# nahomes-15/pointclouds-rs

Hardware: NVIDIA B200
Metric: sor_normals_points_per_sec (higher is better)
Workload: dtype f32

## Files before the change

pointclouds_rs_b200/csrc/grid_build.cu:

```cuda
#include "pcr_internal.cuh"

#include <algorithm>
#include <cstring>
#include <chrono>
#include <cmath>

namespace pcr {

namespace {

constexpr int kBuildThreads = 256;
constexpr int kItems = 4;

using FrameStats = CloudStats;

struct ProbeStats {
    double sum_log_own, sum_log_super;
};

static inline float ordered_f32(unsigned u) {
    unsigned b = (u & 0x80000000u) ? (u & 0x7fffffffu) : ~u;
    float f;
    memcpy(&f, &b, 4);
    return f;
// ... 220 lines not shown
}

struct TombLevels {
    float4 *sorted[4];
    uint32_t n[4];
    int levels;
};
__global__ void __launch_bounds__(256) tombstone_kernel(TombLevels t, const uint8_t *__restrict__ keep) {
    PCR_GRID_DEP_SYNC();
    const uint32_t i = blockIdx.x * blockDim.x + threadIdx.x;
    for (int l = 0; l < t.levels; l++) {
        if (i >= t.n[l]) continue;
        float4 p = t.sorted[l][i];
        if (!keep[__float_as_uint(p.w)]) {
            const float qnan = __int_as_float(0x7fc00000);
            p.x = p.y = p.z = qnan;
            t.sorted[l][i] = p;
        }
    }
}

constexpr int kScanThreads = 256;
constexpr int kScanItems = 16;
constexpr int kScanTile = kScanThreads * kScanItems;

__device__ __forceinline__ uint32_t block_sum_u32(uint32_t v, uint32_t *sh) {
    v = __reduce_add_sync(PCR_FULL, v);
    if ((threadIdx.x & 31) == 0) sh[threadIdx.x >> 5] = v;
    __syncthreads();
    uint32_t t = 0;
    if (threadIdx.x < kScanThreads / 32) t = sh[threadIdx.x];
    if (threadIdx.x < 32) t = __reduce_add_sync(PCR_FULL, t);
    if (threadIdx.x == 0) sh[0] = t;
    __syncthreads();
    t = sh[0];
    __syncthreads();
    return t;
}

__global__ void __launch_bounds__(kScanThreads) scan_tile_sums_kernel(const uint32_t *__restrict__ data, size_t n,
                                                                      uint32_t *__restrict__ tile_sums) {
    __shared__ uint32_t sh[kScanThreads / 32];
    size_t base = (size_t)blockIdx.x * kScanTile;
    uint32_t s = 0;
#pragma unroll
    for (int it = 0; it < kScanItems; it++) {
        size_t i = base + it * kScanThreads + threadIdx.x;
        if (i < n) s += data[i];
    }
    s = block_sum_u32(s, sh);
    if (threadIdx.x == 0) tile_sums[blockIdx.x] = s;
}

constexpr unsigned long long kScanAgg = 1ull << 32, kScanPre = 2ull << 32;

__device__ __forceinline__ uint4 scan_load4(const uint32_t *data, size_t i, size_t n, bool vec) {
    if (vec && i + 3 < n) return *reinterpret_cast<const uint4 *>(data + i);
    uint4 v;
    v.x = i < n ? data[i] : 0u;
    v.y = i + 1 < n ? data[i + 1] : 0u;
    v.z = i + 2 < n ? data[i + 2] : 0u;
    v.w = i + 3 < n ? data[i + 3] : 0u;
    return v;
}

__device__ __forceinline__ void scan_store4(uint32_t *data, size_t i, size_t n, bool vec, uint4 v) {
    if (vec && i + 3 < n) {
        *reinterpret_cast<uint4 *>(data + i) = v;
        return;
    }
    if (i < n) data[i] = v.x;
    if (i + 1 < n) data[i + 1] = v.y;
    if (i + 2 < n) data[i + 2] = v.z;
    if (i + 3 < n) data[i + 3] = v.w;
}

__device__ __forceinline__ uint32_t scan_lookback_warp0(unsigned long long *state, uint32_t tile, uint32_t epoch, uint32_t total, int lane) {
    const unsigned long long tag = (unsigned long long)epoch << 34;
    volatile unsigned long long *vs = state;
    uint32_t pre = 0;
    if (tile > 0) {
        if (lane == 0) vs[tile] = tag | kScanAgg | total;
        long long look = (long long)tile - 1;
        for (;;) {
            const long long t = look - lane;
            const bool need = t >= 0;
            unsigned long long sv = 0;
            uint32_t polls = 0;
            bool ready;
            do {
                if (need) sv = vs[t];
                ready = !need || ((sv >> 34) == epoch && ((sv >> 32) & 3ull) != 0);
                if (++polls > (1u << 26)) __trap();
            } while (!__all_sync(PCR_FULL, ready));
            const unsigned pm = __ballot_sync(PCR_FULL, need && ((sv >> 32) & 3ull) == 2ull);
            const int stop = pm ? __ffs(pm) - 1 : 32;
            pre += __reduce_add_sync(PCR_FULL, (need && lane <= stop) ? (uint32_t)sv : 0u);
            if (pm || look < 32) break;
            look -= 32;
        }
    }
    if (lane == 0) vs[tile] = tag | kScanPre | (uint32_t)(pre + total);
    return pre;
}

__global__ void __launch_bounds__(kScanThreads) scan_lookback_kernel(uint32_t *__restrict__ data, size_t n,
                                                                     unsigned long long *state, uint32_t *ticket,
                                                                     uint32_t epoch, uint32_t tiles, int vec) {
    constexpr int kWarps = kScanThreads / 32, kRows = kScanItems / 4;
    __shared__ uint32_t s_tile, s_pre;
    __shared__ uint32_t warp_tot[kWarps];
    PCR_GRID_DEP_SYNC();
    if (threadIdx.x == 0) s_tile = atomicAdd(ticket, 1u);
    __syncthreads();
    const uint32_t tile = s_tile;
    if (tile >= tiles) return;
    const int lane = threadIdx.x & 31, w = threadIdx.x >> 5;
    const size_t wbase = (size_t)tile * kScanTile + (size_t)w * (kScanItems * 32);
    uint4 v[kRows];
    uint32_t ex[kRows];
    uint32_t carry = 0;
#pragma unroll
    for (int r = 0; r < kRows; r++) {
        v[r] = scan_load4(data, wbase + (size_t)r * 128 + lane * 4, n, vec != 0);
        const uint32_t s = v[r].x + v[r].y + v[r].z + v[r].w;
        uint32_t incl = s;
#pragma unroll
        for (int o = 1; o < 32; o <<= 1) {
            uint32_t u = __shfl_up_sync(PCR_FULL, incl, o);
            if (lane >= o) incl += u;
        }
        ex[r] = carry + incl - s;
        carry += __shfl_sync(PCR_FULL, incl, 31);
    }
    if (lane == 0) warp_tot[w] = carry;
    __syncthreads();
    uint32_t woff = 0, total = 0;
#pragma unroll
    for (int j = 0; j < kWarps; j++) {
        const uint32_t t = warp_tot[j];
        if (j < w) woff += t;
        total += t;
    }
    if (w == 0) {
        const uint32_t pre = scan_lookback_warp0(state, tile, epoch, total, lane);
        if (lane == 0) s_pre = pre;
    }
    __syncthreads();
    const uint32_t base = s_pre + woff;
#pragma unroll
    for (int r = 0; r < kRows; r++) {
        uint4 o;
        o.x = base + ex[r];
        o.y = o.x + v[r].x;
        o.z = o.y + v[r].y;
        o.w = o.z + v[r].z;
// ... 4 lines not shown

__global__ void __launch_bounds__(kScanThreads) scan_apply_u64_kernel(const uint32_t *__restrict__ in,
                                                                      uint64_t *__restrict__ out, size_t n,
                                                                      const uint32_t *__restrict__ tile_sums) {
    __shared__ unsigned long long sh64[kScanThreads / 32];
    __shared__ unsigned long long warp_off[kScanThreads / 32];
    unsigned long long pre = 0;
    for (uint32_t t = threadIdx.x; t < blockIdx.x; t += kScanThreads) pre += tile_sums[t];
    for (int o = 16; o > 0; o >>= 1) pre += __shfl_xor_sync(PCR_FULL, pre, o);
    if ((threadIdx.x & 31) == 0) sh64[threadIdx.x >> 5] = pre;
    __syncthreads();
    pre = 0;
    for (int i = 0; i < kScanThreads / 32; i++) pre += sh64[i];
    __syncthreads();
    size_t base = (size_t)blockIdx.x * kScanTile + (size_t)threadIdx.x * kScanItems;
    uint32_t v[kScanItems];
    unsigned long long tsum = 0;
#pragma unroll
    for (int it = 0; it < kScanItems; it++) {
        size_t i = base + it;
        v[it] = i < n ? in[i] : 0u;
        tsum += v[it];
    }
    unsigned long long incl = tsum;
    const int lane = threadIdx.x & 31, w = threadIdx.x >> 5;
#pragma unroll
    for (int o = 1; o < 32; o <<= 1) {
        unsigned long long u = __shfl_up_sync(PCR_FULL, incl, o);
        if (lane >= o) incl += u;
    }
    if (lane == 31) warp_off[w] = incl;
    __syncthreads();
    if (threadIdx.x == 0) {
        unsigned long long acc = 0;
        for (int i = 0; i < kScanThreads / 32; i++) {
            unsigned long long t = warp_off[i];
            warp_off[i] = acc;
            acc += t;
        }
    }
    __syncthreads();
    unsigned long long run = pre + warp_off[w] + (incl - tsum);
#pragma unroll
    for (int it = 0; it < kScanItems; it++) {
        size_t i = base + it;
        if (i < n) out[i] = run;
        run += v[it];
        if (i + 1 == n) out[n] = run;
    }
}

}

static int exclusive_scan_u32_with(Ctx *ctx, uint32_t *d_data, size_t n, DevBuf &scratch, uint32_t &scan_epoch) {
    if (n == 0) return PCR_OK;
    const size_t tiles = (n + kScanTile - 1) / kScanTile;
    const size_t cap_before = scratch.cap;
    PCR_TRY(ensure(ctx, scratch, 16 + tiles * sizeof(unsigned long long)));
    if (scratch.cap != cap_before || scan_epoch >= (1u << 30) - 2) {
        PCR_CUDA(ctx, cudaMemsetAsync(scratch.p, 0, scratch.cap, ctx->stream));
        scan_epoch = 0;
    }
    const uint32_t epoch = ++scan_epoch;
    uint32_t *ticket = (uint32_t *)scratch.p;
    unsigned long long *state = (unsigned long long *)((char *)scratch.p + 16);
    const int vec = ((uintptr_t)d_data & 15) == 0;
    PCR_CUDA(ctx, launch_chained(scan_lookback_kernel, dim3((unsigned)tiles), dim3(kScanThreads), 0, ctx->stream, d_data, n, state, ticket, epoch,
                                 (uint32_t)tiles, vec));
    ctx->launches++;
    return PCR_OK;
}

int exclusive_scan_u32_dev(Ctx *ctx, uint32_t *d_data, size_t n) { return exclusive_scan_u32_with(ctx, d_data, n, ctx->b_scan, ctx->scan_epoch); }

int exclusive_scan_u64_from_u32_dev(Ctx *ctx, const uint32_t *d_in, uint64_t *d_out, size_t n) {
    if (n == 0) {
        PCR_CUDA(ctx, cudaMemsetAsync(d_out, 0, sizeof(uint64_t), ctx->stream));
        return PCR_OK;
    }
    size_t tiles = (n + kScanTile - 1) / kScanTile;
    PCR_TRY(ensure(ctx, ctx->b_misc2, tiles * sizeof(uint32_t)));
    uint32_t *tile_sums = (uint32_t *)ctx->b_misc2.p;
    scan_tile_sums_kernel<<<(unsigned)tiles, kScanThreads, 0, ctx->stream>>>(d_in, n, tile_sums);
    PCR_LAUNCH_CHECK(ctx);
    scan_apply_u64_kernel<<<(unsigned)tiles, kScanThreads, 0, ctx->stream>>>(d_in, d_out, n, tile_sums);
    PCR_LAUNCH_CHECK(ctx);
    return PCR_OK;
}

namespace {

constexpr uint64_t kMaxCellsPerFrame = 1ull << 24;
constexpr uint64_t kMaxCellsTotal = 1ull << 27;

struct FrameBox {
    double mn[3], ext[3];
    uint32_t count;
};

double occupancy_target(size_t k_hint, bool self_knn) {
    double k = k_hint ? (double)k_hint : 10.0;
    static const bool tile_off = [] {
        const char *e = getenv("PCR_KNN_TILE");
        return e && !strcmp(e, "0");
    }();
    double scale = self_knn && !tile_off && k_hint <= 24 ? 0.5 : 0.25;
    if (const char *e = getenv("PCR_OCC_SCALE")) scale = atof(e);
    return std::min(64.0, std::max(2.0, scale * k));
}

double initial_cell(const FrameBox &b, double target) {
    if (b.count == 0) return 1.0;
    double e[3] = {b.ext[0], b.ext[1], b.ext[2]};
    std::sort(e, e + 3);
    double tiny = std::max(e[2] * 1e-6, 1e-30);
    double vol = std::max(e[0], tiny) * std::max(e[1], tiny) * std::max(e[2], tiny);
    double area = std::max(e[1], tiny) * std::max(e[2], tiny);
    double h3 = std::cbrt(vol * target / b.count);
// ... 403 lines not shown
```

pointclouds_rs_b200/csrc/pcr_internal.cuh:

```cuda
#pragma once
#include <cstdlib>

#include <cuda_runtime.h>
#include <math.h>
#include <stdint.h>
#include <stdio.h>
#include <string.h>

#include <string>
#include <vector>

#include "../../include/pcr_b200.h"

namespace pcr {

struct GridDesc {
    double o[3];
    double h, inv_h;
    int32_t dims[3];
    int32_t ax[3];
    uint32_t cell_base;
    uint32_t n_cells;
    uint32_t pt_begin;
    uint32_t pt_end;
// ... 169 lines not shown

struct CloudStats {
    unsigned mn[3], mx[3];
    unsigned count;
    unsigned valid;
};

struct BuildOpts {
    const CloudStats *known_stats = nullptr;
    size_t k_hint = 0;
    bool self_knn = false;
    int n_frames = 1;
    const uint64_t *frame_offsets = nullptr;
    const uint8_t *d_mask = nullptr;
    bool transient = false;
};
int index_build_dev(Ctx *ctx, const float *dx, const float *dy, const float *dz, size_t n,
                    const BuildOpts &opts, Index **out);
void index_free(Index *ix);
int index_coarser_level(Index *ix, Index **out);
int index_finer_level(Index *ix, Index **out);

int knn_queries_dev(Index *ix, const float *dqx, const float *dqy, const float *dqz, size_t nq,
                    size_t k, uint32_t *d_idx, float *d_dist, uint32_t *d_counts);
struct SorLists {
    size_t K = 0;
    size_t stride = 0;
    uint32_t *lists = nullptr;
    uint8_t *cnt = nullptr;
    uint32_t *fallback = nullptr;
    bool initialised = false;
};
int sor_mean_dist_dev(Index *ix, size_t k, float *d_mean_d, const SorLists *keep_lists = nullptr, bool allow_shard = false);
int normals_from_lists_dev(Index *ix, size_t k, const float vp[3], const SorLists &sl, const uint8_t *d_keep, float *d_nx, float *d_ny,
                           float *d_nz,
                           const unsigned long long *d_kept0 = nullptr, unsigned long long *h_kept0 = nullptr, bool early = false);
int normals_early_fork(Ctx *ctx);
int normals_early_from_lists_dev(Index *ix, size_t k, const float vp[3], const SorLists &sl, float *d_nx, float *d_ny, float *d_nz, bool *launched);
int normals_dev(Index *ix, size_t k, const float vp[3], float *d_nx, float *d_ny, float *d_nz,
                const uint8_t *d_mask, bool allow_shard = false);
bool query_sharding_active(const Ctx *ctx, const Index *ix);
int index_shard_queries(Index *ix);
int index_apply_mask_dev(Index *ix, const uint8_t *d_keep);
int radius_count_dev(Index *ix, const float *dqx, const float *dqy, const float *dqz, size_t nq,
                     float radius, uint32_t *d_counts);
int radius_fill_dev(Index *ix, const float *dqx, const float *dqy, const float *dqz, size_t nq,
                    float radius, const uint64_t *d_offsets, uint32_t *d_idx);

int sor_threshold_mask_dev(Ctx *ctx, const float *d_mean_d, const uint32_t *d_frame_off ,
                           int n_frames, size_t n, float std_mul, uint8_t *d_keep, float *d_stats,
                           unsigned long long *d_kept, bool kept_zeroed = false );

int exclusive_scan_u32_dev(Ctx *ctx, uint32_t *d_data, size_t n_plus_1);
int exclusive_scan_u64_from_u32_dev(Ctx *ctx, const uint32_t *d_in, uint64_t *d_out, size_t n);

struct IcpArgs {
    const float *d_sx, *d_sy, *d_sz;
    size_t ns;
    const float *d_tx, *d_ty, *d_tz;
    size_t nt;
    const float *d_nx, *d_ny, *d_nz;
    pcr_icp_params params;
};
int icp_dev(Ctx *ctx, const IcpArgs &a, pcr_icp_result *result);
struct IcpBatchArgs {
    const float *d_x, *d_y, *d_z;
    size_t n;
    const uint64_t *frame_offsets;
    size_t n_frames;
    const float *d_nx, *d_ny, *d_nz;
    const uint32_t *pairs;
    size_t n_pairs;
    pcr_icp_params params;
};
int icp_batch_dev(Ctx *ctx, const IcpBatchArgs &a, pcr_icp_result *results);
int find_correspondences_dev(Index *target, const float *dsx, const float *dsy, const float *dsz,
                             size_t ns, float max_distance, uint32_t *d_tgt, float *d_dist);
int apply_transform_dev(Ctx *ctx, const float *dx, const float *dy, const float *dz, size_t n,
                        const float R[9], const float t[3], float *ox, float *oy, float *oz);

int cluster_labels_dev(Ctx *ctx, const float *dx, const float *dy, const float *dz, size_t n, float threshold, uint32_t *d_labels,
                       const uint32_t *d_frame_off = nullptr, int n_frames = 1);
size_t clusters_from_labels(const uint32_t *labels, size_t n, size_t min_size, size_t max_size, uint32_t *offsets, uint32_t *indices,
                            std::vector<uint32_t> &scratch);
int cluster_labels_batch_dev(Ctx *ctx, const float *dx, const float *dy, const float *dz, const uint64_t *frame_offsets, size_t n_frames,
                             float threshold, uint32_t *d_labels);
int euclidean_cluster_batch_dev(Ctx *ctx, const float *dx, const float *dy, const float *dz, const uint64_t *frame_offsets, size_t n_frames,
                                float threshold, size_t min_size, size_t max_size, uint32_t *d_offsets, uint32_t *d_indices,
                                uint64_t *cluster_offsets, size_t *total);

int voxel_downsample_dev(Ctx *ctx, const float *dx, const float *dy, const float *dz, size_t n, float voxel, float *d_ox, float *d_oy,
                         float *d_oz, size_t *n_out, CloudStats *stats_out = nullptr ,
                         bool allow_guess = true );
int voxel_downsample_batch_dev(Ctx *ctx, const float *dx, const float *dy, const float *dz, const uint64_t *frame_offsets,
                               size_t n_frames, float voxel, float *d_ox, float *d_oy, float *d_oz, uint64_t *out_offsets);
int radix_sort_pairs_dev(Ctx *ctx, unsigned long long **keys, uint32_t **vals, unsigned long long **keys_alt, uint32_t **vals_alt,
                         size_t n, int bits, uint32_t *d_hist);
size_t radix_sort_hist_words(size_t n);
int bits_for(uint64_t range);

int ransac_plane_samples_dev(Ctx *ctx, const float *dx, const float *dy, const float *dz, size_t n, float threshold,
                             const uint32_t *h_samples, size_t m, float model_out[4], uint32_t *d_inliers, size_t *n_inliers);
int ransac_plane_samples_batch_dev(Ctx *ctx, const float *dx, const float *dy, const float *dz, const uint64_t *frame_offsets,
                                   size_t n_frames, float threshold, const uint32_t *h_samples, const uint64_t *sample_offsets,
                                   float *models_out, uint32_t *d_inliers, uint64_t *inlier_offsets);

// ... 34 lines not shown
    cfg.attrs = at;
    cfg.numAttrs = off ? 0 : 1;
    return cudaLaunchKernelEx(&cfg, kernel, static_cast<KArgs>(args)...);
}

#define PCR_FULL 0xffffffffu
#define PCR_EMPTY_KEY 0x7f80000100000000ull

__device__ __forceinline__ float dist2_exact(float ax, float ay, float az, float bx, float by, float bz) {
    float dx = __fsub_rn(ax, bx), dy = __fsub_rn(ay, by), dz = __fsub_rn(az, bz);
    float s = __fmul_rn(dx, dx);
    s = __fadd_rn(s, __fmul_rn(dy, dy));
    s = __fadd_rn(s, __fmul_rn(dz, dz));
    return s;
}

__device__ __forceinline__ unsigned long long make_key(float d2, uint32_t idx) {
    return ((unsigned long long)__float_as_uint(d2) << 32) | idx;
}
__device__ __forceinline__ float key_d2(unsigned long long k) { return __uint_as_float((uint32_t)(k >> 32)); }
__device__ __forceinline__ uint32_t key_idx(unsigned long long k) { return (uint32_t)k; }

__device__ __forceinline__ bool finite3(float a, float b, float c) { return isfinite(a) && isfinite(b) && isfinite(c); }
__device__ __forceinline__ unsigned f32_ordered(float f) {
    unsigned u = __float_as_uint(f);
    return (u & 0x80000000u) ? ~u : (u | 0x80000000u);
}

__device__ __forceinline__ float pick_axis(int ax, float x, float y, float z) { return ax == 0 ? x : (ax == 1 ? y : z); }

__device__ __forceinline__ int cell_coord(const GridDesc &g, int j, float v, double *frac) {
    double t = ((double)v - g.o[j]) * g.inv_h;
    double f = floor(t);
    f = fmin(fmax(f, 0.0), (double)(g.dims[j] - 1));
    if (frac) *frac = t - f;
    return (int)f;
}

__device__ __forceinline__ uint32_t cell_linear(const GridDesc &g, int c0, int c1, int c2) {
    return g.cell_base + ((uint32_t)c0 * (uint32_t)g.dims[1] + (uint32_t)c1) * (uint32_t)g.dims[2] + (uint32_t)c2;
}

__device__ __forceinline__ int frame_of(const uint32_t *__restrict__ off, int n_frames, uint32_t i) {
    if (n_frames <= 1) return 0;
    int lo = 0, hi = n_frames - 1;
    while (lo < hi) {
        int mid = (lo + hi + 1) >> 1;
        if (off[mid] <= i) lo = mid;
        else hi = mid - 1;
    }
    return lo;
}

#endif

}
```

pointclouds_rs_b200/csrc/voxel.cu:

```cuda
#include "pcr_internal.cuh"

#include <algorithm>

namespace pcr {

namespace {

constexpr int kSortRounds = 8;
constexpr int kSortTile = 32 * kSortRounds;
constexpr int kSortWarps = 4;

struct VoxHeader {
    unsigned mn_c[3], mx[3];
    unsigned count;
    unsigned outside;
    unsigned total;
    unsigned tall;
    unsigned pad[6];
};
constexpr uint32_t kTallColumn = 256;
constexpr uint32_t kLocalColumn = 32;
static_assert(sizeof(VoxHeader) == 64, "header layout");

struct VoxRange {
// ... 196 lines not shown
        return;
    }
    if (vid[i + 1] != vid[i]) start[vid[i]] = i;
}

__global__ void __launch_bounds__(128) vox_mean_kernel(const float *__restrict__ x, const float *__restrict__ y, const float *__restrict__ z,
                                                       const uint32_t *__restrict__ vals, const uint32_t *__restrict__ start,
                                                       const uint32_t *__restrict__ n_vox_dev, float *__restrict__ ox,
                                                       float *__restrict__ oy, float *__restrict__ oz) {
    const uint32_t v = blockIdx.x * blockDim.x + threadIdx.x;
    if (v >= *n_vox_dev) return;
    const uint32_t b = start[v], e = start[v + 1];
    float sx = 0.f, sy = 0.f, sz = 0.f;
    for (uint32_t i = b; i < e; i++) {
        const uint32_t p = vals[i];
        sx = __fadd_rn(sx, x[p]);
        sy = __fadd_rn(sy, y[p]);
        sz = __fadd_rn(sz, z[p]);
    }
    const float denom = (float)(e - b);
    ox[v] = __fdiv_rn(sx, denom);
    oy[v] = __fdiv_rn(sy, denom);
    oz[v] = __fdiv_rn(sz, denom);
}

__global__ void __launch_bounds__(256) vox_col_count_kernel(const float *__restrict__ x, const float *__restrict__ y,
                                                            const float *__restrict__ z, size_t n, float voxel, int mn0, int mn1,
                                                            int mn2, unsigned long long nx, unsigned long long ny,
                                                            unsigned long long nz, uint32_t nyc, int ys, uint32_t *__restrict__ count,
                                                            uint32_t *__restrict__ col_of, uint32_t *__restrict__ rank_of,
                                                            uint32_t *__restrict__ outside) {
    const size_t i = (size_t)blockIdx.x * blockDim.x + threadIdx.x;
    if (i >= n) return;
    const float px = x[i], py = y[i], pz = z[i];
    if (!finite3(px, py, pz)) {
        col_of[i] = 0xffffffffu;
        return;
    }
    const int kx = vox_cell(px, voxel), ky = vox_cell(py, voxel), kz = vox_cell(pz, voxel);
    if ((unsigned long long)((long long)kx - mn0) >= nx || (unsigned long long)((long long)ky - mn1) >= ny ||
        (unsigned long long)((long long)kz - mn2) >= nz) {
        col_of[i] = 0xffffffffu;
        *outside = 1u;
        return;
    }
    const uint32_t col = (uint32_t)(kx - mn0) * nyc + ((uint32_t)(ky - mn1) >> ys);
    col_of[i] = col;
    rank_of[i] = atomicAdd(&count[col], 1u);
}

__global__ void __launch_bounds__(256) vox_col_scatter_kernel(const float *__restrict__ y, const float *__restrict__ z, size_t n,
                                                              float voxel, int mn1, int mn2, int ys,
                                                              const uint32_t *__restrict__ start, const uint32_t *__restrict__ col_of,
                                                              const uint32_t *__restrict__ rank_of, unsigned long long *__restrict__ members) {
    PCR_GRID_DEP_SYNC();
    const size_t i = (size_t)blockIdx.x * blockDim.x + threadIdx.x;
    if (i >= n) return;
    const uint32_t col = col_of[i];
    if (col == 0xffffffffu) return;
    const uint32_t ylo = (uint32_t)(vox_cell(y[i], voxel) - mn1) & ((1u << ys) - 1u);
    const uint32_t hi = (ys ? ylo << (32 - ys) : 0u) | (uint32_t)(vox_cell(z[i], voxel) - mn2);
    members[start[col] + rank_of[i]] = ((unsigned long long)hi << 32) | (uint32_t)i;
}

__global__ void __launch_bounds__(256) vox_col_sort_kernel(const uint32_t *__restrict__ col_of, const uint32_t *__restrict__ rank_of,
                                                           size_t n, const uint32_t *__restrict__ start,
                                                           unsigned long long *__restrict__ members, uint32_t *__restrict__ nvox,
                                                           unsigned *__restrict__ tall) {
    PCR_GRID_DEP_SYNC();
    const size_t i = (size_t)blockIdx.x * blockDim.x + threadIdx.x;
    if (i >= n) return;
    const uint32_t c = col_of[i];
    if (c == 0xffffffffu || rank_of[i] != 0u) return;
    const uint32_t b = start[c], e = start[c + 1], m = e - b;
    if (m > kTallColumn) {
        *tall = 1u;
        return;
    }
    unsigned long long *a = members + b;
    if (m == 1) {
        nvox[b] = 1u;
        return;
    }
    if (m <= kLocalColumn) {
        unsigned long long loc[kLocalColumn];
        for (uint32_t j0 = 0; j0 < m; j0 += 8) {
            unsigned long long t[8];
#pragma unroll
            for (int u = 0; u < 8; u++) t[u] = a[min(j0 + u, m - 1)];
#pragma unroll
            for (int u = 0; u < 8; u++)
                if (j0 + u < m) loc[j0 + u] = t[u];
        }
        for (uint32_t i = 1; i < m; i++) {
            const unsigned long long v = loc[i];
            uint32_t j = i;
            while (j > 0 && loc[j - 1] > v) {
                loc[j] = loc[j - 1];
                j--;
            }
            loc[j] = v;
        }
        uint32_t nv = 1;
        a[0] = loc[0];
        for (uint32_t i = 1; i < m; i++) {
            a[i] = loc[i];
            nv += (uint32_t)(loc[i] >> 32) != (uint32_t)(loc[i - 1] >> 32) ? 1u : 0u;
        }
        nvox[b] = nv;
        return;
    } else {
        for (uint32_t s0 = m / 2; s0-- > 0;) {
            uint32_t root = s0;
            for (;;) {
                uint32_t ch = 2 * root + 1;
// ... 65 lines not shown
                cnt = 0;
                cur = kz;
            }
            sx = __fadd_rn(sx, X[u]);
            sy = __fadd_rn(sy, Y[u]);
            sz = __fadd_rn(sz, Z[u]);
            cnt++;
        }
    }
    const float denom = (float)cnt;
    ox[v] = __fdiv_rn(sx, denom);
    oy[v] = __fdiv_rn(sy, denom);
    oz[v] = __fdiv_rn(sz, denom);
}

__global__ void __launch_bounds__(256) vox_out_stats_kernel(const float *__restrict__ x, const float *__restrict__ y,
                                                            const float *__restrict__ z, const uint32_t *__restrict__ d_n,
                                                            VoxHeader *hdr) {
    PCR_GRID_DEP_SYNC();
    const uint32_t n = *d_n;
    if (blockIdx.x == 0 && threadIdx.x == 0) hdr->total = n;
    unsigned mn_c[3] = {0u, 0u, 0u}, mx[3] = {0u, 0u, 0u}, cnt = 0;
    for (uint32_t i = blockIdx.x * blockDim.x + threadIdx.x; i < n; i += gridDim.x * blockDim.x) {
        const float px = x[i], py = y[i], pz = z[i];
        if (!finite3(px, py, pz)) continue;
        const unsigned u[3] = {f32_ordered(px), f32_ordered(py), f32_ordered(pz)};
        for (int a = 0; a < 3; a++) {
            mn_c[a] = max(mn_c[a], ~u[a]);
            mx[a] = max(mx[a], u[a]);
        }
        cnt++;
    }
    for (int a = 0; a < 3; a++) {
        mn_c[a] = __reduce_max_sync(PCR_FULL, mn_c[a]);
        mx[a] = __reduce_max_sync(PCR_FULL, mx[a]);
    }
    cnt = __reduce_add_sync(PCR_FULL, cnt);
    __shared__ unsigned s_mn[3], s_mx[3], s_cnt;
    if (threadIdx.x == 0) {
        s_mn[0] = s_mn[1] = s_mn[2] = 0u;
        s_mx[0] = s_mx[1] = s_mx[2] = 0u;
        s_cnt = 0;
    }
    __syncthreads();
    if ((threadIdx.x & 31) == 0 && cnt) {
        for (int a = 0; a < 3; a++) {
            atomicMax(&s_mn[a], mn_c[a]);
            atomicMax(&s_mx[a], mx[a]);
        }
        atomicAdd(&s_cnt, cnt);
    }
    __syncthreads();
    if (threadIdx.x == 0 && s_cnt) {
        for (int a = 0; a < 3; a++) {
            atomicMax(&hdr->mn_c[a], s_mn[a]);
            atomicMax(&hdr->mx[a], s_mx[a]);
        }
        atomicAdd(&hdr->count, s_cnt);
    }
}

__global__ void __launch_bounds__(256) vox_frame_starts_kernel(const unsigned long long *__restrict__ keys, const uint32_t *__restrict__ vals,
                                                               uint32_t m, int fshift ,
                                                               const uint32_t *__restrict__ frame_off, int n_frames,
                                                               const uint32_t *__restrict__ vid, uint32_t *__restrict__ out_off) {
    const uint32_t i = blockIdx.x * blockDim.x + threadIdx.x;
    if (i > m) return;
    auto frame = [&](uint32_t j) { return fshift >= 0 ? (int)(keys[j] >> fshift) : frame_of(frame_off, n_frames, vals[j]); };
    const int hi = i < m ? frame(i) : n_frames;
    const int lo = i > 0 ? frame(i - 1) : -1;
    for (int f = lo + 1; f <= hi; f++) out_off[f] = vid[i];
}

}

int bits_for(uint64_t range) {
    int b = 0;
    while (b < 64 && (1ull << b) < range) b++;
    return b;
}

size_t radix_sort_hist_words(size_t n) { return (size_t)256 * ((n + kSortTile - 1) / kSortTile) + 1; }

int radix_sort_pairs_dev(Ctx *ctx, unsigned long long **keys, uint32_t **vals, unsigned long long **keys_alt, uint32_t **vals_alt,
                         size_t n, int bits, uint32_t *d_hist ) {
    if (n == 0) return PCR_OK;
    const uint32_t n_tiles = (uint32_t)((n + kSortTile - 1) / kSortTile);
    const unsigned blocks = (n_tiles + kSortWarps - 1) / kSortWarps;
    for (int shift = 0; shift < bits; shift += 8) {
        sort_hist_kernel<<<blocks, 32 * kSortWarps, 0, ctx->stream>>>(*keys, n, shift, n_tiles, d_hist);
        PCR_LAUNCH_CHECK(ctx);
        PCR_TRY(exclusive_scan_u32_dev(ctx, d_hist, (size_t)256 * n_tiles + 1));
        sort_scatter_kernel<<<blocks, 32 * kSortWarps, 0, ctx->stream>>>(*keys, *vals, n, shift, n_tiles, d_hist, *keys_alt, *vals_alt);
        PCR_LAUNCH_CHECK(ctx);
        std::swap(*keys, *keys_alt);
        std::swap(*vals, *vals_alt);
    }
    return PCR_OK;
}

int voxel_downsample_dev(Ctx *ctx, const float *dx, const float *dy, const float *dz, size_t n, float voxel, float *d_ox, float *d_oy,
                         float *d_oz, size_t *n_out, CloudStats *stats_out, bool allow_guess) {
    *n_out = 0;
    if (stats_out) stats_out->valid = 0;
    if (n == 0) return PCR_OK;
    if (n > 0x7fffffffull) return fail(ctx, PCR_ERR_UNSUPPORTED, "clouds above 2^31 points are not supported");
    cudaStream_t st = ctx->stream;
    TimeScope ts(ctx, kTagOther);
    PCR_TRY(ensure(ctx, ctx->b_small, 4096));
    PCR_TRY(ensure_pinned(ctx, 4096));
    VoxRange *d_range = (VoxRange *)ctx->b_small.p;
    uint32_t *d_nvox = (uint32_t *)((char *)ctx->b_small.p + 256);
    VoxRange *h_range = (VoxRange *)ctx->pinned;
    auto &vc = ctx->vox_cache;
    static const bool no_guess = getenv("PCR_NO_VOXEL_GUESS") != nullptr;
    const bool guessed = allow_guess && !no_guess && ctx->frame_stream && vc.valid && vc.voxel == voxel && vc.uses < 32;
    uint32_t m;
    if (guessed) {
        vc.uses++;
        for (int a = 0; a < 3; a++) {
            h_range->mn[a] = vc.mn[a];
            h_range->mx[a] = vc.mx[a];
        }
        m = (uint32_t)n;
    } else {
        vox_init_kernel<<<1, 1, 0, st>>>(d_range, 1);
        PCR_LAUNCH_CHECK(ctx);
        const unsigned bx = (unsigned)std::min<size_t>((n + 255) / 256, (size_t)ctx->sm_count * 2);
        vox_range_kernel<<<bx, 256, 0, st>>>(dx, dy, dz, nullptr, n, voxel, d_range);
        PCR_LAUNCH_CHECK(ctx);
        PCR_CUDA(ctx, cudaMemcpyAsync(h_range, d_range, sizeof(VoxRange), cudaMemcpyDeviceToHost, st));
        PCR_MARK("voxel: wait for range");
        PCR_CUDA(ctx, cudaStreamSynchronize(st));
        PCR_MARK("voxel: got range");
        m = h_range->finite;
        if (m == 0) return PCR_OK;
        vc.valid = false;
        if (ctx->frame_stream) {
            bool ok = true;
            for (int a = 0; a < 3; a++) {
                const long long ext = (long long)h_range->mx[a] - (long long)h_range->mn[a] + 1;
                const long long pad = std::max<long long>(2, ext >> vc.pad_shift);
                const long long lo = (long long)h_range->mn[a] - pad, hi = (long long)h_range->mx[a] + pad;
                if (lo < -2147483647ll || hi > 2147483646ll) ok = false;
                vc.mn[a] = (int)lo;
                vc.mx[a] = (int)hi;
            }
            vc.valid = ok;
            vc.voxel = voxel;
            vc.uses = 0;
        }
    }
    {
        const uint64_t nx = (uint64_t)((int64_t)h_range->mx[0] - (int64_t)h_range->mn[0]) + 1;
        const uint64_t ny = (uint64_t)((int64_t)h_range->mx[1] - (int64_t)h_range->mn[1]) + 1;
        const uint64_t nz = (uint64_t)((int64_t)h_range->mx[2] - (int64_t)h_range->mn[2]) + 1;
        int ys = 0;
        static const int ys_max = getenv("PCR_VOXEL_YS") ? atoi(getenv("PCR_VOXEL_YS")) : 0;
        while (ys < ys_max && nz < (1ull << (32 - (ys + 1))) && nx * ((ny + (2ull << ys) - 1) >> (ys + 1)) >= (uint64_t)m) ys++;
        while (ys < 4 && nz < (1ull << (32 - (ys + 1))) && nx * ((ny + (1ull << ys) - 1) >> ys) > (1ull << 24)) ys++;
        const uint64_t nyc64 = (ny + (1ull << ys) - 1) >> ys;
        const uint64_t n_cols64 = nx * nyc64;
        static const bool no_cols = getenv("PCR_VOXEL_RADIX") != nullptr;
        if (!no_cols && nx < (1ull << 31) && ny < (1ull << 31) && nz < (1ull << (32 - ys)) && n_cols64 <= (1ull << 24) &&
            n_cols64 <= 64ull * m + 65536ull) {
            const uint32_t n_cols = (uint32_t)n_cols64;
            const size_t tab = (sizeof(uint32_t) * ((size_t)n_cols + 1) + 15) & ~(size_t)15;
            const size_t tab_v = (sizeof(uint32_t) * ((size_t)n + 1) + 15) & ~(size_t)15;
            const size_t o_count = sizeof(VoxHeader), o_nvox = o_count + tab;
            const size_t o_col = (o_nvox + tab_v + 15) & ~(size_t)15;
            const size_t o_rank = o_col + sizeof(uint32_t) * n;
            const size_t o_mem = (o_rank + sizeof(uint32_t) * n + 15) & ~(size_t)15;
            PCR_TRY(ensure(ctx, ctx->b_table, o_mem + sizeof(unsigned long long) * n));
            char *base = (char *)ctx->b_table.p;
            VoxHeader *d_hdr = (VoxHeader *)base;
            uint32_t *count = (uint32_t *)(base + o_count), *nvox = (uint32_t *)(base + o_nvox);
            uint32_t *col_of = (uint32_t *)(base + o_col), *rank_of = (uint32_t *)(base + o_rank);
            unsigned long long *members = (unsigned long long *)(base + o_mem);
            PCR_CUDA(ctx, cudaMemsetAsync(base, 0, o_nvox + tab_v, st));
            const unsigned nbp = (unsigned)((n + 255) / 256);
            vox_col_count_kernel<<<nbp, 256, 0, st>>>(dx, dy, dz, n, voxel, h_range->mn[0], h_range->mn[1], h_range->mn[2], nx, ny, nz,
                                                      (uint32_t)nyc64, ys, count, col_of, rank_of, &d_hdr->outside);
            PCR_LAUNCH_CHECK(ctx);
            PCR_TRY(exclusive_scan_u32_dev(ctx, count, (size_t)n_cols + 1));
            PCR_CUDA(ctx, launch_chained(vox_col_scatter_kernel, dim3(nbp), dim3(256), 0, st, dy, dz, n, voxel, h_range->mn[1], h_range->mn[2], ys,
                                         count, col_of, rank_of, members));
            PCR_CUDA(ctx, launch_chained(vox_col_sort_kernel, dim3(nbp), dim3(256), 0, st, col_of, rank_of, n, count, members, nvox, &d_hdr->tall));
            ctx->launches += 2;
            PCR_TRY(exclusive_scan_u32_dev(ctx, nvox, n + 1));
            PCR_CUDA(ctx, launch_chained(vox_col_emit_kernel, dim3(nbp), dim3(256), 0, st, dx, dy, dz, col_of, rank_of, n, count, nvox, members, d_ox,
                                         d_oy, d_oz));
            ctx->launches++;
            PCR_CUDA(ctx, launch_chained(vox_out_stats_kernel, dim3((unsigned)ctx->sm_count), dim3(256), 0, st, d_ox, d_oy, d_oz, nvox + n, d_hdr));
            ctx->launches++;
            VoxHeader *mail = (VoxHeader *)((uint32_t *)ctx->pinned + 64);
            PCR_CUDA(ctx, cudaMemcpyAsync(mail, d_hdr, sizeof(VoxHeader), cudaMemcpyDeviceToHost, st));
            PCR_MARK("voxel: wait for count");
            PCR_CUDA(ctx, cudaStreamSynchronize(st));
            PCR_MARK("voxel: got count");
            if (guessed) (mail->outside ? ctx->stat_vox_misses : ctx->stat_vox_hits)++;
            if (guessed && mail->outside) {
                vc.valid = false;
                vc.pad_shift = std::max(2, vc.pad_shift - 1);
                return voxel_downsample_dev(ctx, dx, dy, dz, n, voxel, d_ox, d_oy, d_oz, n_out, stats_out, false);
            }
            const bool tall = mail->tall != 0;
            if (tall && guessed) {
                vc.valid = false;
                return voxel_downsample_dev(ctx, dx, dy, dz, n, voxel, d_ox, d_oy, d_oz, n_out, stats_out, false);
            }
            if (!tall) *n_out = mail->total;
            if (!tall && stats_out) {
                for (int a = 0; a < 3; a++) {
                    stats_out->mn[a] = ~mail->mn_c[a];
                    stats_out->mx[a] = mail->mx[a];
                }
                stats_out->count = mail->count;
                stats_out->valid = 1;
            }
            if (!tall) return PCR_OK;
        }
    }
    if (guessed) {
        vc.valid = false;
        return voxel_downsample_dev(ctx, dx, dy, dz, n, voxel, d_ox, d_oy, d_oz, n_out, stats_out, false);
    }
    int bits[3];
    for (int a = 0; a < 3; a++) bits[a] = bits_for((uint64_t)((int64_t)h_range->mx[a] - (int64_t)h_range->mn[a]) + 1);
    const int total_bits = bits[0] + bits[1] + bits[2];
    const bool packed = total_bits <= 63;

    const size_t n_tiles = (n + kSortTile - 1) / kSortTile;
    const size_t need = 2 * sizeof(unsigned long long) * n + sizeof(uint32_t) * (2 * n + 256 * n_tiles + 1 + 2 * (n + 1)) + 1024;
    PCR_TRY(ensure(ctx, ctx->b_table, need));
    char *p = (char *)ctx->b_table.p;
    unsigned long long *kA = (unsigned long long *)p;
    p += sizeof(unsigned long long) * n;
    unsigned long long *kB = (unsigned long long *)p;
    p += sizeof(unsigned long long) * n;
    uint32_t *vA = (uint32_t *)p;
    p += sizeof(uint32_t) * n;
    uint32_t *vB = (uint32_t *)p;
    p += sizeof(uint32_t) * n;
    uint32_t *hist = (uint32_t *)p;
    p += sizeof(uint32_t) * (256 * n_tiles + 1);
    uint32_t *vid = (uint32_t *)p;
    p += sizeof(uint32_t) * (n + 1);
// ... 136 lines not shown
```

Baseline: 264.4 million.

## Replace voxel column pipeline with bucketed tile sort-emit kernel using decoupled lookback

Makes a new default voxel downsampling path that bins points into coarser xy buckets and sorts each ~1024-point tile in shared memory. A single kernel then segments voxels, averages them, assigns output offsets through a decoupled lookback scan and accumulates bounds stats. It replaces the separate sort, second scan, emit and stats kernels, cutting launches and global passes. The cost is an extra bounds array written during scatter and an O(bucket size) rank loop per point. Tiles over capacity set the tall flag and fall back.

```diff
diff --git a/pointclouds_rs_b200/csrc/grid_build.cu b/pointclouds_rs_b200/csrc/grid_build.cu
--- a/pointclouds_rs_b200/csrc/grid_build.cu
+++ b/pointclouds_rs_b200/csrc/grid_build.cu
@@ -296,8 +296,6 @@
     if (threadIdx.x == 0) tile_sums[blockIdx.x] = s;
 }
 
-constexpr unsigned long long kScanAgg = 1ull << 32, kScanPre = 2ull << 32;
-
 __device__ __forceinline__ uint4 scan_load4(const uint32_t *data, size_t i, size_t n, bool vec) {
     if (vec && i + 3 < n) return *reinterpret_cast<const uint4 *>(data + i);
     uint4 v;
@@ -317,35 +315,6 @@
     if (i + 1 < n) data[i + 1] = v.y;
     if (i + 2 < n) data[i + 2] = v.z;
     if (i + 3 < n) data[i + 3] = v.w;
-}
-
-__device__ __forceinline__ uint32_t scan_lookback_warp0(unsigned long long *state, uint32_t tile, uint32_t epoch, uint32_t total, int lane) {
-    const unsigned long long tag = (unsigned long long)epoch << 34;
-    volatile unsigned long long *vs = state;
-    uint32_t pre = 0;
-    if (tile > 0) {
-        if (lane == 0) vs[tile] = tag | kScanAgg | total;
-        long long look = (long long)tile - 1;
-        for (;;) {
-            const long long t = look - lane;
-            const bool need = t >= 0;
-            unsigned long long sv = 0;
-            uint32_t polls = 0;
-            bool ready;
-            do {
-                if (need) sv = vs[t];
-                ready = !need || ((sv >> 34) == epoch && ((sv >> 32) & 3ull) != 0);
-                if (++polls > (1u << 26)) __trap();
-            } while (!__all_sync(PCR_FULL, ready));
-            const unsigned pm = __ballot_sync(PCR_FULL, need && ((sv >> 32) & 3ull) == 2ull);
-            const int stop = pm ? __ffs(pm) - 1 : 32;
-            pre += __reduce_add_sync(PCR_FULL, (need && lane <= stop) ? (uint32_t)sv : 0u);
-            if (pm || look < 32) break;
-            look -= 32;
-        }
-    }
-    if (lane == 0) vs[tile] = tag | kScanPre | (uint32_t)(pre + total);
-    return pre;
 }
 
 __global__ void __launch_bounds__(kScanThreads) scan_lookback_kernel(uint32_t *__restrict__ data, size_t n,
@@ -456,18 +425,29 @@
 
 }
 
-static int exclusive_scan_u32_with(Ctx *ctx, uint32_t *d_data, size_t n, DevBuf &scratch, uint32_t &scan_epoch) {
-    if (n == 0) return PCR_OK;
-    const size_t tiles = (n + kScanTile - 1) / kScanTile;
+static int lookback_scratch_with(Ctx *ctx, size_t tiles, DevBuf &scratch, uint32_t &scan_epoch, LookbackScratch *lb) {
     const size_t cap_before = scratch.cap;
     PCR_TRY(ensure(ctx, scratch, 16 + tiles * sizeof(unsigned long long)));
     if (scratch.cap != cap_before || scan_epoch >= (1u << 30) - 2) {
         PCR_CUDA(ctx, cudaMemsetAsync(scratch.p, 0, scratch.cap, ctx->stream));
         scan_epoch = 0;
     }
-    const uint32_t epoch = ++scan_epoch;
-    uint32_t *ticket = (uint32_t *)scratch.p;
-    unsigned long long *state = (unsigned long long *)((char *)scratch.p + 16);
+    lb->epoch = ++scan_epoch;
+    lb->ticket = (uint32_t *)scratch.p;
+    lb->state = (unsigned long long *)((char *)scratch.p + 16);
+    return PCR_OK;
+}
+
+int lookback_scratch(Ctx *ctx, size_t tiles, LookbackScratch *lb) { return lookback_scratch_with(ctx, tiles, ctx->b_scan, ctx->scan_epoch, lb); }
+
+static int exclusive_scan_u32_with(Ctx *ctx, uint32_t *d_data, size_t n, DevBuf &scratch, uint32_t &scan_epoch) {
+    if (n == 0) return PCR_OK;
+    const size_t tiles = (n + kScanTile - 1) / kScanTile;
+    LookbackScratch lb;
+    PCR_TRY(lookback_scratch_with(ctx, tiles, scratch, scan_epoch, &lb));
+    const uint32_t epoch = lb.epoch;
+    uint32_t *ticket = lb.ticket;
+    unsigned long long *state = lb.state;
     const int vec = ((uintptr_t)d_data & 15) == 0;
     PCR_CUDA(ctx, launch_chained(scan_lookback_kernel, dim3((unsigned)tiles), dim3(kScanThreads), 0, ctx->stream, d_data, n, state, ticket, epoch,
                                  (uint32_t)tiles, vec));
diff --git a/pointclouds_rs_b200/csrc/pcr_internal.cuh b/pointclouds_rs_b200/csrc/pcr_internal.cuh
--- a/pointclouds_rs_b200/csrc/pcr_internal.cuh
+++ b/pointclouds_rs_b200/csrc/pcr_internal.cuh
@@ -245,6 +245,12 @@
                            unsigned long long *d_kept, bool kept_zeroed = false );
 
 int exclusive_scan_u32_dev(Ctx *ctx, uint32_t *d_data, size_t n_plus_1);
+struct LookbackScratch {
+    uint32_t *ticket;
+    unsigned long long *state;
+    uint32_t epoch;
+};
+int lookback_scratch(Ctx *ctx, size_t tiles, LookbackScratch *lb);
 int exclusive_scan_u64_from_u32_dev(Ctx *ctx, const uint32_t *d_in, uint64_t *d_out, size_t n);
 
 struct IcpArgs {
@@ -385,6 +391,37 @@
     return lo;
 }
 
+constexpr unsigned long long kScanAgg = 1ull << 32, kScanPre = 2ull << 32;
+
+__device__ __forceinline__ uint32_t scan_lookback_warp0(unsigned long long *state, uint32_t tile, uint32_t epoch, uint32_t total, int lane) {
+    const unsigned long long tag = (unsigned long long)epoch << 34;
+    volatile unsigned long long *vs = state;
+    uint32_t pre = 0;
+    if (tile > 0) {
+        if (lane == 0) vs[tile] = tag | kScanAgg | total;
+        long long look = (long long)tile - 1;
+        for (;;) {
+            const long long t = look - lane;
+            const bool need = t >= 0;
+            unsigned long long sv = 0;
+            uint32_t polls = 0;
+            bool ready;
+            do {
+                if (need) sv = vs[t];
+                ready = !need || ((sv >> 34) == epoch && ((sv >> 32) & 3ull) != 0);
+                if (++polls > (1u << 26)) __trap();
+            } while (!__all_sync(PCR_FULL, ready));
+            const unsigned pm = __ballot_sync(PCR_FULL, need && ((sv >> 32) & 3ull) == 2ull);
+            const int stop = pm ? __ffs(pm) - 1 : 32;
+            pre += __reduce_add_sync(PCR_FULL, (need && lane <= stop) ? (uint32_t)sv : 0u);
+            if (pm || look < 32) break;
+            look -= 32;
+        }
+    }
+    if (lane == 0) vs[tile] = tag | kScanPre | (uint32_t)(pre + total);
+    return pre;
+}
+
 #endif
 
 }
diff --git a/pointclouds_rs_b200/csrc/voxel.cu b/pointclouds_rs_b200/csrc/voxel.cu
--- a/pointclouds_rs_b200/csrc/voxel.cu
+++ b/pointclouds_rs_b200/csrc/voxel.cu
@@ -272,7 +272,8 @@
 __global__ void __launch_bounds__(256) vox_col_scatter_kernel(const float *__restrict__ y, const float *__restrict__ z, size_t n,
                                                               float voxel, int mn1, int mn2, int ys,
                                                               const uint32_t *__restrict__ start, const uint32_t *__restrict__ col_of,
-                                                              const uint32_t *__restrict__ rank_of, unsigned long long *__restrict__ members) {
+                                                              const uint32_t *__restrict__ rank_of, unsigned long long *__restrict__ members,
+                                                              unsigned long long *__restrict__ bounds ) {
     PCR_GRID_DEP_SYNC();
     const size_t i = (size_t)blockIdx.x * blockDim.x + threadIdx.x;
     if (i >= n) return;
@@ -280,7 +281,9 @@
     if (col == 0xffffffffu) return;
     const uint32_t ylo = (uint32_t)(vox_cell(y[i], voxel) - mn1) & ((1u << ys) - 1u);
     const uint32_t hi = (ys ? ylo << (32 - ys) : 0u) | (uint32_t)(vox_cell(z[i], voxel) - mn2);
-    members[start[col] + rank_of[i]] = ((unsigned long long)hi << 32) | (uint32_t)i;
+    const uint32_t b = start[col], slot = b + rank_of[i];
+    members[slot] = ((unsigned long long)hi << 32) | (uint32_t)i;
+    if (bounds) bounds[slot] = ((unsigned long long)start[col + 1] << 32) | b;
 }
 
 __global__ void __launch_bounds__(256) vox_col_sort_kernel(const uint32_t *__restrict__ col_of, const uint32_t *__restrict__ rank_of,
@@ -452,6 +455,178 @@
     }
     __syncthreads();
     if (threadIdx.x == 0 && s_cnt) {
+        for (int a = 0; a < 3; a++) {
+            atomicMax(&hdr->mn_c[a], s_mn[a]);
+            atomicMax(&hdr->mx[a], s_mx[a]);
+        }
+        atomicAdd(&hdr->count, s_cnt);
+    }
+}
+
+constexpr int kBktThreads = 256;
+constexpr uint32_t kBktTile = 1024;
+constexpr uint32_t kBktCap = 2048;
+constexpr int kBktPer = (int)(kBktCap / kBktThreads);
+static_assert(kBktCap % kBktThreads == 0, "bucket tile layout");
+
+__global__ void __launch_bounds__(kBktThreads) vox_bkt_sort_emit_kernel(
+    const float *__restrict__ x, const float *__restrict__ y, const float *__restrict__ z, const unsigned long long *__restrict__ bounds,
+    const uint32_t *__restrict__ start, uint32_t n_buckets, const unsigned long long *__restrict__ members, float *__restrict__ ox,
+    float *__restrict__ oy, float *__restrict__ oz, unsigned long long *lb_state, uint32_t *lb_ticket, uint32_t lb_epoch, uint32_t tiles,
+    VoxHeader *hdr) {
+    __shared__ unsigned long long s_key[kBktCap];
+    __shared__ float s_x[kBktCap], s_y[kBktCap], s_z[kBktCap];
+    __shared__ uint8_t s_head[kBktCap];
+    __shared__ uint32_t s_tile, s_range[2], s_pre, s_wsum[kBktThreads / 32];
+    __shared__ unsigned s_mn[3], s_mx[3], s_cnt;
+    PCR_GRID_DEP_SYNC();
+    const int tid = threadIdx.x, lane = tid & 31, w = tid >> 5;
+    if (tid == 0) {
+        s_tile = atomicAdd(lb_ticket, 1u);
+        s_mn[0] = s_mn[1] = s_mn[2] = 0u;
+        s_mx[0] = s_mx[1] = s_mx[2] = 0u;
+        s_cnt = 0;
+    }
+    __syncthreads();
+    const uint32_t tile = s_tile;
+    if (tile >= tiles) return;
+    if (tid < 2) {
+        const uint32_t M = start[n_buckets];
+        const uint64_t p = (uint64_t)(tile + tid) * kBktTile;
+        uint32_t a = M;
+        if (p < M) {
+            const unsigned long long bd = bounds[p];
+            a = (uint32_t)bd == (uint32_t)p ? (uint32_t)p : (uint32_t)(bd >> 32);
+        }
+        s_range[tid] = a;
+    }
+    __syncthreads();
+    const uint32_t lo = s_range[0];
+    uint32_t len = s_range[1] - lo;
+    if (len > kBktCap) {
+        if (tid == 0) hdr->tall = 1u;
+        len = 0;
+    }
+    unsigned long long key[kBktPer];
+    uint32_t bs[kBktPer], be[kBktPer];
+    float X[kBktPer], Y[kBktPer], Z[kBktPer];
+#pragma unroll
+    for (int k = 0; k < kBktPer; k++) {
+        const uint32_t j = tid + k * kBktThreads;
+        key[k] = 0ull;
+        bs[k] = be[k] = 0u;
+        if (j < len) {
+            key[k] = members[lo + j];
+            const unsigned long long bd = bounds[lo + j];
+            bs[k] = (uint32_t)bd - lo;
+            be[k] = (uint32_t)(bd >> 32) - lo;
+        }
+    }
+#pragma unroll
+    for (int k = 0; k < kBktPer; k++) {
+        const uint32_t j = tid + k * kBktThreads;
+        X[k] = Y[k] = Z[k] = 0.f;
+        if (j < len) {
+            s_key[j] = key[k];
+            const uint32_t p = (uint32_t)key[k];
+            X[k] = x[p];
+            Y[k] = y[p];
+            Z[k] = z[p];
+        }
+    }
+    __syncthreads();
+#pragma unroll
+    for (int k = 0; k < kBktPer; k++) {
+        const uint32_t j = tid + k * kBktThreads;
+        if (j < len) {
+            const uint32_t vk = (uint32_t)(key[k] >> 32);
+            uint32_t r = 0, same = 0;
+            for (uint32_t q = bs[k]; q < be[k]; q++) {
+                const unsigned long long o = s_key[q];
+                const bool less = o < key[k];
+                r += less ? 1u : 0u;
+                same += (less && (uint32_t)(o >> 32) == vk) ? 1u : 0u;
+            }
+            const uint32_t pos = bs[k] + r;
+            s_x[pos] = X[k];
+            s_y[pos] = Y[k];
+            s_z[pos] = Z[k];
+            s_head[pos] = same == 0 ? 1 : 0;
+        }
+    }
+    __syncthreads();
+    const uint32_t c0 = (uint32_t)tid * kBktPer;
+    uint32_t nh = 0;
+#pragma unroll
+    for (int k = 0; k < kBktPer; k++) nh += (c0 + k < len && s_head[c0 + k]) ? 1u : 0u;
+    uint32_t incl = nh;
+#pragma unroll
+    for (int o = 1; o < 32; o <<= 1) {
+        const uint32_t u = __shfl_up_sync(PCR_FULL, incl, o);
+        if (lane >= o) incl += u;
+    }
+    if (lane == 31) s_wsum[w] = incl;
+    __syncthreads();
+    uint32_t woff = 0, total = 0;
+#pragma unroll
+    for (int q = 0; q < kBktThreads / 32; q++) {
+        const uint32_t t = s_wsum[q];
+        if (q < w) woff += t;
+        total += t;
+    }
+    if (w == 0) {
+        const uint32_t pre = scan_lookback_warp0(lb_state, tile, lb_epoch, total, lane);
+        if (lane == 0) {
+            s_pre = pre;
+            if (tile == tiles - 1) {
+                hdr->total = pre + total;
+                *lb_ticket = 0;
+            }
+        }
+    }
+    __syncthreads();
+    uint32_t v = s_pre + woff + incl - nh;
+    unsigned mn_c[3] = {0u, 0u, 0u}, mx[3] = {0u, 0u, 0u}, cnt = 0;
+    for (int k = 0; k < kBktPer; k++) {
+        const uint32_t h = c0 + k;
+        if (h >= len) break;
+        if (!s_head[h]) continue;
+        float sx = __fadd_rn(0.f, s_x[h]), sy = __fadd_rn(0.f, s_y[h]), sz = __fadd_rn(0.f, s_z[h]);
+        uint32_t e = h + 1;
+        for (; e < len && !s_head[e]; e++) {
+            sx = __fadd_rn(sx, s_x[e]);
+            sy = __fadd_rn(sy, s_y[e]);
+            sz = __fadd_rn(sz, s_z[e]);
+        }
+        const float denom = (float)(e - h);
+        const float mxv = __fdiv_rn(sx, denom), myv = __fdiv_rn(sy, denom), mzv = __fdiv_rn(sz, denom);
+        ox[v] = mxv;
+        oy[v] = myv;
+        oz[v] = mzv;
+        v++;
+        if (finite3(mxv, myv, mzv)) {
+            const unsigned u3[3] = {f32_ordered(mxv), f32_ordered(myv), f32_ordered(mzv)};
+            for (int a = 0; a < 3; a++) {
+                mn_c[a] = max(mn_c[a], ~u3[a]);
+                mx[a] = max(mx[a], u3[a]);
+            }
+            cnt++;
+        }
+    }
+    for (int a = 0; a < 3; a++) {
+        mn_c[a] = __reduce_max_sync(PCR_FULL, mn_c[a]);
+        mx[a] = __reduce_max_sync(PCR_FULL, mx[a]);
+    }
+    cnt = __reduce_add_sync(PCR_FULL, cnt);
+    if (lane == 0 && cnt) {
+        for (int a = 0; a < 3; a++) {
+            atomicMax(&s_mn[a], mn_c[a]);
+            atomicMax(&s_mx[a], mx[a]);
+        }
+        atomicAdd(&s_cnt, cnt);
+    }
+    __syncthreads();
+    if (tid == 0 && s_cnt) {
         for (int a = 0; a < 3; a++) {
             atomicMax(&hdr->mn_c[a], s_mn[a]);
             atomicMax(&hdr->mx[a], s_mx[a]);
@@ -555,44 +730,85 @@
         const uint64_t nx = (uint64_t)((int64_t)h_range->mx[0] - (int64_t)h_range->mn[0]) + 1;
         const uint64_t ny = (uint64_t)((int64_t)h_range->mx[1] - (int64_t)h_range->mn[1]) + 1;
         const uint64_t nz = (uint64_t)((int64_t)h_range->mx[2] - (int64_t)h_range->mn[2]) + 1;
-        int ys = 0;
-        static const int ys_max = getenv("PCR_VOXEL_YS") ? atoi(getenv("PCR_VOXEL_YS")) : 0;
-        while (ys < ys_max && nz < (1ull << (32 - (ys + 1))) && nx * ((ny + (2ull << ys) - 1) >> (ys + 1)) >= (uint64_t)m) ys++;
-        while (ys < 4 && nz < (1ull << (32 - (ys + 1))) && nx * ((ny + (1ull << ys) - 1) >> ys) > (1ull << 24)) ys++;
-        const uint64_t nyc64 = (ny + (1ull << ys) - 1) >> ys;
-        const uint64_t n_cols64 = nx * nyc64;
         static const bool no_cols = getenv("PCR_VOXEL_RADIX") != nullptr;
-        if (!no_cols && nx < (1ull << 31) && ny < (1ull << 31) && nz < (1ull << (32 - ys)) && n_cols64 <= (1ull << 24) &&
-            n_cols64 <= 64ull * m + 65536ull) {
-            const uint32_t n_cols = (uint32_t)n_cols64;
-            const size_t tab = (sizeof(uint32_t) * ((size_t)n_cols + 1) + 15) & ~(size_t)15;
-            const size_t tab_v = (sizeof(uint32_t) * ((size_t)n + 1) + 15) & ~(size_t)15;
-            const size_t o_count = sizeof(VoxHeader), o_nvox = o_count + tab;
-            const size_t o_col = (o_nvox + tab_v + 15) & ~(size_t)15;
-            const size_t o_rank = o_col + sizeof(uint32_t) * n;
-            const size_t o_mem = (o_rank + sizeof(uint32_t) * n + 15) & ~(size_t)15;
-            PCR_TRY(ensure(ctx, ctx->b_table, o_mem + sizeof(unsigned long long) * n));
-            char *base = (char *)ctx->b_table.p;
-            VoxHeader *d_hdr = (VoxHeader *)base;
-            uint32_t *count = (uint32_t *)(base + o_count), *nvox = (uint32_t *)(base + o_nvox);
-            uint32_t *col_of = (uint32_t *)(base + o_col), *rank_of = (uint32_t *)(base + o_rank);
-            unsigned long long *members = (unsigned long long *)(base + o_mem);
-            PCR_CUDA(ctx, cudaMemsetAsync(base, 0, o_nvox + tab_v, st));
-            const unsigned nbp = (unsigned)((n + 255) / 256);
-            vox_col_count_kernel<<<nbp, 256, 0, st>>>(dx, dy, dz, n, voxel, h_range->mn[0], h_range->mn[1], h_range->mn[2], nx, ny, nz,
-                                                      (uint32_t)nyc64, ys, count, col_of, rank_of, &d_hdr->outside);
-            PCR_LAUNCH_CHECK(ctx);
-            PCR_TRY(exclusive_scan_u32_dev(ctx, count, (size_t)n_cols + 1));
-            PCR_CUDA(ctx, launch_chained(vox_col_scatter_kernel, dim3(nbp), dim3(256), 0, st, dy, dz, n, voxel, h_range->mn[1], h_range->mn[2], ys,
-                                         count, col_of, rank_of, members));
-            PCR_CUDA(ctx, launch_chained(vox_col_sort_kernel, dim3(nbp), dim3(256), 0, st, col_of, rank_of, n, count, members, nvox, &d_hdr->tall));
-            ctx->launches += 2;
-            PCR_TRY(exclusive_scan_u32_dev(ctx, nvox, n + 1));
-            PCR_CUDA(ctx, launch_chained(vox_col_emit_kernel, dim3(nbp), dim3(256), 0, st, dx, dy, dz, col_of, rank_of, n, count, nvox, members, d_ox,
-                                         d_oy, d_oz));
-            ctx->launches++;
-            PCR_CUDA(ctx, launch_chained(vox_out_stats_kernel, dim3((unsigned)ctx->sm_count), dim3(256), 0, st, d_ox, d_oy, d_oz, nvox + n, d_hdr));
-            ctx->launches++;
+        static const bool columns = getenv("PCR_VOXEL_COLUMNS") != nullptr;
+        const unsigned nbp = (unsigned)((n + 255) / 256);
+        VoxHeader *d_hdr = nullptr;
+        if (!no_cols && !columns) {
+            const uint64_t want = std::max<uint64_t>((uint64_t)m / 2, 4096);
+            int s = 0;
+            while (s < 24 && nx * ((ny + (1ull << s) - 1) >> s) > want) s++;
+            const uint64_t nyb64 = (ny + (1ull << s) - 1) >> s;
+            const uint64_t n_bkt64 = nx * nyb64;
+            if (nx < (1ull << 31) && ny < (1ull << 31) && nz < (1ull << (32 - s)) && n_bkt64 <= (1ull << 24) &&
+                n_bkt64 <= 64ull * m + 65536ull) {
+                const uint32_t n_bkt = (uint32_t)n_bkt64;
+                const size_t o_count = sizeof(VoxHeader);
+                const size_t o_col = (o_count + sizeof(uint32_t) * ((size_t)n_bkt + 1) + 15) & ~(size_t)15;
+                const size_t o_rank = o_col + sizeof(uint32_t) * n;
+                const size_t o_mem = (o_rank + sizeof(uint32_t) * n + 15) & ~(size_t)15;
+                const size_t o_bnd = o_mem + sizeof(unsigned long long) * n;
+                PCR_TRY(ensure(ctx, ctx->b_table, o_bnd + sizeof(unsigned long long) * n));
+                char *base = (char *)ctx->b_table.p;
+                d_hdr = (VoxHeader *)base;
+                uint32_t *count = (uint32_t *)(base + o_count);
+                uint32_t *col_of = (uint32_t *)(base + o_col), *rank_of = (uint32_t *)(base + o_rank);
+                unsigned long long *members = (unsigned long long *)(base + o_mem), *bounds = (unsigned long long *)(base + o_bnd);
+                const uint32_t tiles = (uint32_t)((n + kBktTile - 1) / kBktTile);
+                PCR_CUDA(ctx, cudaMemsetAsync(base, 0, o_count + sizeof(uint32_t) * ((size_t)n_bkt + 1), st));
+                vox_col_count_kernel<<<nbp, 256, 0, st>>>(dx, dy, dz, n, voxel, h_range->mn[0], h_range->mn[1], h_range->mn[2], nx, ny, nz,
+                                                          (uint32_t)nyb64, s, count, col_of, rank_of, &d_hdr->outside);
+                PCR_LAUNCH_CHECK(ctx);
+                PCR_TRY(exclusive_scan_u32_dev(ctx, count, (size_t)n_bkt + 1));
+                LookbackScratch lb;
+                PCR_TRY(lookback_scratch(ctx, tiles, &lb));
+                PCR_CUDA(ctx, launch_chained(vox_col_scatter_kernel, dim3(nbp), dim3(256), 0, st, dy, dz, n, voxel, h_range->mn[1], h_range->mn[2], s,
+                                             count, col_of, rank_of, members, bounds));
+                PCR_CUDA(ctx, launch_chained(vox_bkt_sort_emit_kernel, dim3(tiles), dim3(kBktThreads), 0, st, dx, dy, dz, bounds, count, n_bkt, members,
+                                             d_ox, d_oy, d_oz, lb.state, lb.ticket, lb.epoch, tiles, d_hdr));
+                ctx->launches += 2;
+            }
+        }
+        if (!no_cols && columns) {
+            int ys = 0;
+            static const int ys_max = getenv("PCR_VOXEL_YS") ? atoi(getenv("PCR_VOXEL_YS")) : 0;
+            while (ys < ys_max && nz < (1ull << (32 - (ys + 1))) && nx * ((ny + (2ull << ys) - 1) >> (ys + 1)) >= (uint64_t)m) ys++;
+            while (ys < 4 && nz < (1ull << (32 - (ys + 1))) && nx * ((ny + (1ull << ys) - 1) >> ys) > (1ull << 24)) ys++;
+            const uint64_t nyc64 = (ny + (1ull << ys) - 1) >> ys;
+            const uint64_t n_cols64 = nx * nyc64;
+            if (nx < (1ull << 31) && ny < (1ull << 31) && nz < (1ull << (32 - ys)) && n_cols64 <= (1ull << 24) &&
+                n_cols64 <= 64ull * m + 65536ull) {
+                const uint32_t n_cols = (uint32_t)n_cols64;
+                const size_t tab = (sizeof(uint32_t) * ((size_t)n_cols + 1) + 15) & ~(size_t)15;
+                const size_t tab_v = (sizeof(uint32_t) * ((size_t)n + 1) + 15) & ~(size_t)15;
+                const size_t o_count = sizeof(VoxHeader), o_nvox = o_count + tab;
+                const size_t o_col = (o_nvox + tab_v + 15) & ~(size_t)15;
+                const size_t o_rank = o_col + sizeof(uint32_t) * n;
+                const size_t o_mem = (o_rank + sizeof(uint32_t) * n + 15) & ~(size_t)15;
+                PCR_TRY(ensure(ctx, ctx->b_table, o_mem + sizeof(unsigned long long) * n));
+                char *base = (char *)ctx->b_table.p;
+                d_hdr = (VoxHeader *)base;
+                uint32_t *count = (uint32_t *)(base + o_count), *nvox = (uint32_t *)(base + o_nvox);
+                uint32_t *col_of = (uint32_t *)(base + o_col), *rank_of = (uint32_t *)(base + o_rank);
+                unsigned long long *members = (unsigned long long *)(base + o_mem);
+                PCR_CUDA(ctx, cudaMemsetAsync(base, 0, o_nvox + tab_v, st));
+                vox_col_count_kernel<<<nbp, 256, 0, st>>>(dx, dy, dz, n, voxel, h_range->mn[0], h_range->mn[1], h_range->mn[2], nx, ny, nz,
+                                                          (uint32_t)nyc64, ys, count, col_of, rank_of, &d_hdr->outside);
+                PCR_LAUNCH_CHECK(ctx);
+                PCR_TRY(exclusive_scan_u32_dev(ctx, count, (size_t)n_cols + 1));
+                PCR_CUDA(ctx, launch_chained(vox_col_scatter_kernel, dim3(nbp), dim3(256), 0, st, dy, dz, n, voxel, h_range->mn[1], h_range->mn[2], ys,
+                                             count, col_of, rank_of, members, (unsigned long long *)nullptr));
+                PCR_CUDA(ctx, launch_chained(vox_col_sort_kernel, dim3(nbp), dim3(256), 0, st, col_of, rank_of, n, count, members, nvox, &d_hdr->tall));
+                ctx->launches += 2;
+                PCR_TRY(exclusive_scan_u32_dev(ctx, nvox, n + 1));
+                PCR_CUDA(ctx, launch_chained(vox_col_emit_kernel, dim3(nbp), dim3(256), 0, st, dx, dy, dz, col_of, rank_of, n, count, nvox, members, d_ox,
+                                             d_oy, d_oz));
+                ctx->launches++;
+                PCR_CUDA(ctx, launch_chained(vox_out_stats_kernel, dim3((unsigned)ctx->sm_count), dim3(256), 0, st, d_ox, d_oy, d_oz, nvox + n, d_hdr));
+                ctx->launches++;
+            }
+        }
+        if (d_hdr) {
             VoxHeader *mail = (VoxHeader *)((uint32_t *)ctx->pinned + 64);
             PCR_CUDA(ctx, cudaMemcpyAsync(mail, d_hdr, sizeof(VoxHeader), cudaMemcpyDeviceToHost, st));
             PCR_MARK("voxel: wait for count");
```

New measurement: 272.3 million (median of 6 runs). 1.03x the previous value.
